# roysubhankar/dwt-domain-adaptation

Hardware: AMD Instinct MI355X
Metric: imgs_per_sec (higher is better)
Workload: dtype bf16; 1 GPU; model=resnet50-dwt-mec-3stream, global_batch=1536, seq_len=224, parallelism=dp1, per_domain_batch=512, group_size=4, whiten_mode=zca

## Files before the change

### dwt_amd/kernels/hip_ops.py

```python
from __future__ import annotations

import warnings
import torch

from . import dispatch

_GEN_G_MAX = 32
_warned = set()


def _whiten_layout(x, c, g):
    if x.dim() == 4 and x.is_contiguous(memory_format=torch.channels_last) \
            and not x.is_contiguous():
        if c % 64 == 0 and (c <= 256 or c % 256 == 0) and g in (2, 4):
            gw = min(c, 256) // g
            if gw > 0 and 256 % gw == 0:
                return "cl"
    return "nchw"


def _bn_cl_supported(c):
    if c % 4 != 0 or (c > 1024 and c % 1024 != 0):
        return False
    nch = min(c, 1024) // 4
    return 256 % nch == 0


def _bn_layout(x, c):
    if x.dim() == 2 and x.is_contiguous() and _bn_cl_supported(c):
        return "cl"
    if x.dim() == 4 and x.is_contiguous(memory_format=torch.channels_last) \
            and not x.is_contiguous() and _bn_cl_supported(c):
        return "cl"
    return "nchw"


def _warn_once(key, msg):
    if key not in _warned:
        _warned.add(key)
        warnings.warn(msg)


def _sync_world():
    import torch.distributed as dist
    if dist.is_available() and dist.is_initialized():
        return dist, dist.get_world_size()
    return None, 1


def _allreduce(t):
    import torch.distributed as dist
    dist.all_reduce(t)
    return t


def _ext():
    return dispatch.ext()


def _f32c(t):
    return t.detach().to(torch.float32).contiguous()


class _HipWhitenMulti(torch.autograd.Function):

    @staticmethod
    def forward(ctx, x, gamma, beta, running_means, running_vars, cfg,
                res=None):
        ext = _ext()
        parts = cfg["parts"]
        g = x.shape[1] // cfg["num_groups"]
        eps, momentum = cfg["eps"], cfg["momentum"]
        training, mode, relu = cfg["training"], cfg["mode"], cfg["relu"]
        track = cfg.get("track_running_stats", True)
        ns_iters = cfg.get("ns_iters", 7)
        use_batch = training or not track

        c = x.shape[1]
        layout = _whiten_layout(x, c, g)
        if layout == "nchw":
            x = x.contiguous()
        n, c, h, w = x.shape
        assert n % parts == 0,             f"batch {n} not divisible by {parts} domain branches"
        b = n // parts
        n_groups = c // g
        ng_all = parts * n_groups
        dev = x.device
        m_count = b * h * w

        has_affine = gamma is not None
        gflat = gamma.detach().reshape(c).contiguous() if has_affine else torch.empty(0, device=dev, dtype=x.dtype)
        bflat = beta.detach().reshape(c).contiguous() if has_affine else torch.empty(0, device=dev, dtype=x.dtype)

        stats_sync = cfg.get("stats_sync", False) and use_batch
        world = 1
        if stats_sync:
            _, world = _sync_world()
        ctx_count = m_count * world

        out = torch.empty_like(x)
        if use_batch:
            acc = torch.zeros(ng_all * (g + g * g), device=dev, dtype=torch.float32)
            mean = torch.empty(parts * c, device=dev, dtype=torch.float32)
            cov = torch.empty(ng_all, g, g, device=dev, dtype=torch.float32)
            if stats_sync:
                if layout == "cl":
                    ext.whiten_stats_partial_cl(x, acc, g, c, m_count, parts)
                else:
                    for p in range(parts):
                        ext.whiten_stats_partial(
                            x[p * b:(p + 1) * b],
                            acc[p * n_groups * (g + g * g):(p + 1) * n_groups * (g + g * g)], g)
                if world > 1:
                    _allreduce(acc)
                ext.whiten_stats_final(acc, mean, cov, g, ng_all, ctx_count)
            elif layout == "cl":
                ext.whiten_stats_cl(x, acc, mean, cov, g, c, m_count, parts)
            else:
                for p in range(parts):
                    ext.whiten_stats(x[p * b:(p + 1) * b],
                                     acc[p * n_groups * (g + g * g):(p + 1) * n_groups * (g + g * g)],
                                     mean[p * c:(p + 1) * c],
                                     cov[p * n_groups:(p + 1) * n_groups], g)
        else:
            mean = torch.stack([_f32c(running_means[p]).reshape(c)
                                for p in range(parts)]).reshape(-1).contiguous()
            cov = torch.stack([_f32c(running_vars[p]).reshape(n_groups, g, g)
                               for p in range(parts)]).reshape(ng_all, g, g).contiguous()
# ... 188 lines not shown
    c = x.shape[1]
    if kind == "whiten":
        return _whiten_layout(x, c, c // cfg["num_groups"]) == "cl"
    return _bn_layout(x, c) == "cl"


def whiten_join(x, identity, gamma, beta, running_means, running_vars, cfg):
    return _HipWhitenJoin.apply(x, identity, gamma, beta, running_means,
                                running_vars, cfg)


def batch_norm_join(x, identity, gamma, beta, running_means, running_vars, cfg):
    return _HipBatchNormJoin.apply(x, identity, gamma, beta, running_means,
                                   running_vars, cfg)


def whiten_multi(x, gamma, beta, running_means, running_vars, cfg):
    g = x.shape[1] // cfg["num_groups"]
    if g > _GEN_G_MAX or x.dtype not in (torch.float32, torch.bfloat16):
        _warn_once(("wh", g, x.dtype),
                   f"dwt_amd: whiten_multi g={g} dtype={x.dtype} uses the "
                   "torch path (HIP kernels cover g <= 32, fp32/bf16)")
        from ..ops.functional import WhitenMulti
        return WhitenMulti.apply(x, gamma, beta, running_means, running_vars, cfg)
    return _HipWhitenMulti.apply(x, gamma, beta, running_means, running_vars, cfg)


class _HipBatchNormMulti(torch.autograd.Function):
    @staticmethod
    def forward(ctx, x, gamma, beta, running_means, running_vars, cfg,
                res=None):
        ext = _ext()
        parts = cfg["parts"]
        eps, momentum = cfg["eps"], cfg["momentum"]
        training, relu = cfg["training"], cfg["relu"]
        track = cfg.get("track_running_stats", True)
        use_batch = training or not track

        spatial = x.dim() == 4
        c = x.shape[1]
        layout = _bn_layout(x, c)
        if layout == "nchw" or x.dim() == 2:
            x = x.contiguous()
        n = x.shape[0]
        assert n % parts == 0,             f"batch {n} not divisible by {parts} domain branches"
        b = n // parts
        dev = x.device
        cnt = (x.numel() // parts) // c

        has_affine = gamma is not None
        gflat = gamma.detach().reshape(c).contiguous() if has_affine else torch.empty(0, device=dev, dtype=x.dtype)
        bflat = beta.detach().reshape(c).contiguous() if has_affine else torch.empty(0, device=dev, dtype=x.dtype)

        stats_sync = cfg.get("stats_sync", False) and use_batch
        world = 1
        if stats_sync:
            _, world = _sync_world()
        cnt_total = cnt * world

        out = torch.empty_like(x)
        if use_batch:
            acc = torch.zeros(parts * 2 * c, device=dev, dtype=torch.float32)
            mean = torch.empty(parts * c, device=dev, dtype=torch.float32)
            istd = torch.empty(parts * c, device=dev, dtype=torch.float32)
            var_unb = torch.empty(parts * c, device=dev, dtype=torch.float32)
            if stats_sync:
                if layout == "cl":
                    ext.bn_stats_partial_cl(x, acc, c, cnt, parts)
                else:
                    for p in range(parts):
                        ext.bn_stats_partial(x[p * b:(p + 1) * b],
                                             acc[p * 2 * c:(p + 1) * 2 * c])
                if world > 1:
                    _allreduce(acc)
                ext.bn_stats_final(acc, mean, istd, var_unb, c, parts,
                                   cnt_total, eps)
            elif layout == "cl":
                ext.bn_stats_cl(x, acc, mean, istd, var_unb, c, cnt, eps, parts)
            else:
                for p in range(parts):
                    ext.bn_stats(x[p * b:(p + 1) * b],
                                 acc[p * 2 * c:(p + 1) * 2 * c],
                                 mean[p * c:(p + 1) * c],
                                 istd[p * c:(p + 1) * c],
                                 var_unb[p * c:(p + 1) * c], eps)
            if training and track and running_means is not None:
                with torch.no_grad():
                    for p in range(parts):
                        rm, rv = running_means[p], running_vars[p]
# ... 116 lines not shown
    @staticmethod
    def forward(ctx, x, identity, gamma, beta, running_means, running_vars,
                cfg):
        ctx.set_materialize_grads(False)
        res = identity.detach()
        y = _HipBatchNormMulti.forward(ctx, x, gamma, beta, running_means,
                                       running_vars, cfg, res=res)
        return y, y.view_as(y)

    @staticmethod
    def backward(ctx, ga, gb):
        if ga is None and gb is None:
            return (None,) * 7
        if ga is None:
            ga, gb = gb, None
        dx, gid, dgamma, dbeta = _HipBatchNormMulti.run_backward(
            ctx, ga, gb, join=True)
        return dx, gid, dgamma, dbeta, None, None, None


def batch_norm_multi(x, gamma, beta, running_means, running_vars, cfg):
    if x.dtype not in (torch.float32, torch.bfloat16):
        from ..ops.functional import BatchNormMulti
        return BatchNormMulti.apply(x, gamma, beta, running_means, running_vars, cfg)
    return _HipBatchNormMulti.apply(x, gamma, beta, running_means, running_vars, cfg)


class _HipMecLoss(torch.autograd.Function):
    @staticmethod
    def forward(ctx, x, y):
        ext = _ext()
        x32 = x.detach().to(torch.float32).contiguous()
        y32 = y.detach().to(torch.float32).contiguous()
        n, k = x32.shape
        lx = torch.empty_like(x32)
        ly = torch.empty_like(y32)
        amin = torch.empty(n, device=x.device, dtype=torch.int32)
        loss = torch.zeros(1, device=x.device, dtype=torch.float32)
        ext.mec_fwd(x32, y32, lx, ly, amin, loss)
        ctx.save_for_backward(lx, ly, amin)
        ctx.dtypes = (x.dtype, y.dtype)
        return loss[0]

    @staticmethod
    def backward(ctx, dloss):
        ext = _ext()
# ... 66 lines not shown
```

### dwt_amd/kernels/src/dwt_kernels.hip

```cpp

#include <torch/extension.h>
#include <ATen/cuda/CUDAContext.h>
#include <hip/hip_runtime.h>

#include <cstdint>

#define DEV_INLINE __device__ __forceinline__

namespace dwt {


DEV_INLINE float ldf(const float* p) { return *p; }
DEV_INLINE float ldf(const c10::BFloat16* p) {
  unsigned short u = *reinterpret_cast<const unsigned short*>(p);
  union { unsigned int i; float f; } v;
  v.i = static_cast<unsigned int>(u) << 16;
  return v.f;
}
DEV_INLINE void stf(float* p, float v) { *p = v; }
DEV_INLINE void stf(c10::BFloat16* p, float v) {
  union { unsigned int i; float f; } u;
  u.f = v;
  unsigned int lsb = (u.i >> 16) & 1u;
  unsigned int rounded = u.i + 0x7fffu + lsb;
// ... 3104 lines not shown
                     0, cur_stream(), q.data_ptr<float>(),
                     target.data_ptr<int64_t>(), gscale.data_ptr<float>(),
                     dx.data_ptr<float>(), N, K);
}

void entropy_bwd(Tensor q, Tensor hper, Tensor gscale, Tensor dx) {
  const int N = q.size(0), K = q.size(1);
  const int64_t total = (int64_t)N * K;
  hipLaunchKernelGGL(dwt::entropy_bwd_kernel,
                     dim3(elementwise_blocks(total, 256)), dim3(256), 0,
                     cur_stream(), q.data_ptr<float>(), hper.data_ptr<float>(),
                     gscale.data_ptr<float>(), dx.data_ptr<float>(), N, K);
}

}

void mfma_gemm(torch::Tensor a, torch::Tensor bt, torch::Tensor bias,
               torch::Tensor out, bool relu, bool has_bias);
void mfma_conv2d_fwd(torch::Tensor x, torch::Tensor wgt, torch::Tensor bias,
                     torch::Tensor out, int64_t N, int64_t H, int64_t W,
                     int64_t Cin, int64_t P, int64_t Q, int64_t Cout,
                     int64_t KH, int64_t KW, int64_t stride, int64_t pad,
                     bool relu, bool has_bias);
void mfma_conv2d_dgrad(torch::Tensor dy, torch::Tensor wd, torch::Tensor dx,
                       int64_t N, int64_t H, int64_t W, int64_t Cin,
                       int64_t P, int64_t Q, int64_t Cdy, int64_t KH,
                       int64_t KW, int64_t stride, int64_t pad);
void mfma_conv2d_wgrad(torch::Tensor dy, torch::Tensor x, torch::Tensor dw,
                       torch::Tensor ws, int64_t N, int64_t H, int64_t W,
                       int64_t Cin, int64_t P, int64_t Q, int64_t Cout,
                       int64_t KH, int64_t KW, int64_t stride, int64_t pad);

PYBIND11_MODULE(TORCH_EXTENSION_NAME, m) {
  m.def("mfma_gemm", &mfma_gemm);
  m.def("mfma_conv2d_fwd", &mfma_conv2d_fwd);
  m.def("mfma_conv2d_dgrad", &mfma_conv2d_dgrad);
  m.def("mfma_conv2d_wgrad", &mfma_conv2d_wgrad);
  m.def("whiten_stats", &whiten_stats);
  m.def("whiten_stats_partial", &whiten_stats_partial);
  m.def("whiten_stats_partial_cl", &whiten_stats_partial_cl);
  m.def("whiten_stats_final", &whiten_stats_final);
  m.def("bn_stats_partial", &bn_stats_partial);
  m.def("bn_stats_partial_cl", &bn_stats_partial_cl);
  m.def("bn_stats_final", &bn_stats_final);
  m.def("whiten_stats_cl", &whiten_stats_cl);
  m.def("whiten_apply_cl", &whiten_apply_cl);
  m.def("whiten_bwd_reduce_cl", &whiten_bwd_reduce_cl);
  m.def("whiten_bwd_apply_cl", &whiten_bwd_apply_cl);
  m.def("bn_stats_cl", &bn_stats_cl);
  m.def("bn_apply_cl", &bn_apply_cl);
  m.def("bn_bwd_reduce_cl", &bn_bwd_reduce_cl);
  m.def("bn_bwd_apply_cl", &bn_bwd_apply_cl);
  m.def("whiten_apply_res_cl", &whiten_apply_res_cl);
  m.def("bn_apply_res_cl", &bn_apply_res_cl);
  m.def("whiten_join_bwd_reduce_cl", &whiten_join_bwd_reduce_cl);
  m.def("bn_join_bwd_reduce_cl", &bn_join_bwd_reduce_cl);
  m.def("matfn_chol_fwd", &matfn_chol_fwd);
  m.def("matfn_chol_bwd", &matfn_chol_bwd);
// ... 26 lines not shown
```

### dwt_amd/kernels/src/mfma_conv.hip

```cpp

#include <torch/extension.h>
#include <ATen/cuda/CUDAContext.h>
#include <hip/hip_runtime.h>

#include <cstdint>

namespace dwtmm {

using bf16 = c10::BFloat16;
typedef __attribute__((ext_vector_type(8))) short short8;
typedef __attribute__((ext_vector_type(4))) float floatx4;

#define DEV_INLINE __device__ __forceinline__

constexpr int BM = 128, BN = 128, BK = 64;
constexpr int THREADS = 256;
constexpr int PAD_HALFS = 8;
constexpr int LDS_PITCH = BK + PAD_HALFS;

struct ConvParams {
  int N, H, W, Cin;
  int P, Q, Cout;
  int KH, KW, stride, pad;
  int64_t M;
// ... 300 lines not shown
        __syncthreads();
      }
    } else {
      __syncthreads();
    }
  }

  const int erow = (lane / 16) * 4;
  const int ecol = lane % 16;
#pragma unroll
  for (int i = 0; i < 4; ++i) {
#pragma unroll
    for (int r = 0; r < 4; ++r) {
      const int64_t m = m0 + wm + i * 16 + erow + r;
      if (m >= cp.M) continue;
#pragma unroll
      for (int j = 0; j < 4; ++j) {
        const int n = n0 + wn + j * 16 + ecol;
        if (n >= cp.Cout) continue;
        float v = acc[i][j][r];
        if (HAS_BIAS) v += bias[n];
        if (RELU) v = fmaxf(v, 0.f);
        *reinterpret_cast<unsigned short*>(out + m * cp.Cout + n) = f_to_bf16(v);
      }
    }
  }
}




constexpr int WBK = 64;
constexpr int WPITCH = WBK;

DEV_INLINE int wswz(int row) { return ((row >> 3) ^ row) & 7; }

template <bool ALIGNED_B, int WT>
__global__ __launch_bounds__(256, WT == 64 ? 4 : 3) void wgrad_splitk_kernel(
    const bf16* __restrict__ dy, const bf16* __restrict__ x,
    float* __restrict__ ws, ConvParams cp, int mtiles, int ntiles,
    int splitk, int64_t klen) {
  constexpr int NP = WT / 64;
  constexpr int NF = WT / 32;
  __shared__ unsigned short lds_a[WT * WPITCH];
  __shared__ unsigned short lds_b[WT * WPITCH];

// ... 361 lines not shown
                                                                   : dwtmm::A_CONV,
                                            decltype(reluc)::value,
                                            decltype(biasc)::value,
                                            decltype(pipec)::value,
                                            decltype(swzc)::value>),
          dim3(mtiles * ntiles), dim3(dwtmm::THREADS), 0, dwtmm_stream(),
          (const c10::BFloat16*)x.data_ptr(), (const c10::BFloat16*)wgt.data_ptr(),
          has_bias ? bias.data_ptr<float>() : nullptr,
          (c10::BFloat16*)out.data_ptr(), cp, mtiles, ntiles);
    };
    if (pipe) { if (swz) launch(std::true_type{}, std::true_type{});
                else launch(std::true_type{}, std::false_type{}); }
    else { if (swz) launch(std::false_type{}, std::true_type{});
           else launch(std::false_type{}, std::false_type{}); }
  };
  auto pick_rb = [&](auto fastc) {
    if (relu) { if (has_bias) run(fastc, std::true_type{}, std::true_type{});
                else run(fastc, std::true_type{}, std::false_type{}); }
    else { if (has_bias) run(fastc, std::false_type{}, std::true_type{});
           else run(fastc, std::false_type{}, std::false_type{}); }
  };
  if (gemm_fast) pick_rb(std::true_type{});
  else pick_rb(std::false_type{});
}


void mfma_conv2d_dgrad(Tensor dy, Tensor wd, Tensor dx, int64_t N, int64_t H,
                       int64_t W, int64_t Cin, int64_t P, int64_t Q,
                       int64_t Cdy, int64_t KH, int64_t KW, int64_t stride,
                       int64_t pad) {
  dwtmm::ConvParams cp{};
  cp.N = N; cp.H = H; cp.W = W; cp.Cin = Cin;
  cp.P = P; cp.Q = Q; cp.Cout = Cin;
  cp.KH = KH; cp.KW = KW; cp.stride = stride; cp.pad = pad;
  cp.Cdy = Cdy;
  cp.M = N * H * W;
  cp.K = KH * KW * Cdy;
  cp.cShift = log2_if_pow2(Cdy);
  const int mtiles = (cp.M + dwtmm::BM - 1) / dwtmm::BM;
  const int ntiles = (Cin + dwtmm::BN - 1) / dwtmm::BN;
  const bool gemm_fast = (KH == 1 && KW == 1 && stride == 1 && pad == 0 &&
                          Cdy % 8 == 0);
  const bool pipe = gemm_fast && cp.K >= 4 * dwtmm::BK;
  const bool swz = gemm_fast && ntiles >= 8 && mtiles * ntiles >= 16;
  auto launch = [&](auto modec, auto pipec, auto swzc) {
    hipLaunchKernelGGL(
// ... 93 lines not shown
```

### dwt_amd/models/resnet_dwt.py

```python
from __future__ import annotations

from typing import Dict, Optional

import torch
import torch.nn as nn

from ..ops.batch_norm import DomainBatchNorm2d
from ..ops.whitening import WhiteningScaleShift
from ..ops.pooling import MaxPool2dDWT, global_avg_pool
from .sites import norm_site


def _conv_cls():
    import os
    if os.environ.get("DWT_AMD_CONV") == "hip":
        from ..ops.mfma import MFMAConv2d
        return MFMAConv2d
    return nn.Conv2d


def conv3x3(cin, cout, stride=1):
    return _conv_cls()(cin, cout, kernel_size=3, stride=stride, padding=1, bias=False)


def conv1x1(cin, cout, stride=1):
    return _conv_cls()(cin, cout, kernel_size=1, stride=stride, bias=False)


def _get(bn_dict: Optional[Dict], key: str):
    if bn_dict is None:
        return None
    return bn_dict.get(key)


def _make_wh_branches(planes, group_size, bn_dict, prefix, mode):
    branches = []
    for _ in range(3):
        rm = _get(bn_dict, f"{prefix}.wh.running_mean")
        rv = _get(bn_dict, f"{prefix}.wh.running_variance")
        branches.append(WhiteningScaleShift(
            planes, group_size,
            running_mean=rm.clone() if rm is not None else None,
            running_variance=rv.clone() if rv is not None else None,
            affine=False, mode=mode))
    g = _get(bn_dict, f"{prefix}.gamma")
    b = _get(bn_dict, f"{prefix}.beta")
    gamma = nn.Parameter(g.clone() if g is not None else torch.ones(planes, 1, 1))
    beta = nn.Parameter(b.clone() if b is not None else torch.zeros(planes, 1, 1))
    return branches, gamma, beta
# ... 39 lines not shown
            site(planes * self.expansion, "bn3")

        self.downsample = downsample
        self.stride = stride
        if downsample is not None:
            dpre = f"layer{layer}.0.downsample_bn"
            if use_wh:
                (self.downsample_bns, self.downsample_bnt, self.downsample_bnt_aug), \
                    self.downsample_gamma, self.downsample_beta = _make_wh_branches(
                        planes * self.expansion, group_size, bn_dict, dpre, whiten_mode)
            else:
                (self.downsample_bns, self.downsample_bnt, self.downsample_bnt_aug), \
                    self.downsample_gamma, self.downsample_beta = _make_bn_branches(
                        planes * self.expansion, bn_dict, dpre)

    def forward(self, x):
        return self.forward_pair(x, x)[0]

    def forward_pair(self, x_main, x_id):
        tr = self.training
        x = x_main
        identity = x_id

        out = self.conv1(x)
        out = norm_site(out, [self.bns1, self.bnt1, self.bnt1_aug],
                        self.gamma1, self.beta1, training=tr, relu=True)
        out = self.conv2(out)
        out = norm_site(out, [self.bns2, self.bnt2, self.bnt2_aug],
                        self.gamma2, self.beta2, training=tr, relu=True)
        out = self.conv3(out)

        if self.downsample is not None:
            identity = self.downsample(x)
            identity = norm_site(
                identity,
                [self.downsample_bns, self.downsample_bnt, self.downsample_bnt_aug],
                self.downsample_gamma, self.downsample_beta, training=tr, relu=False)

        return norm_site(out, [self.bns3, self.bnt3, self.bnt3_aug],
                         self.gamma3, self.beta3, training=tr, relu=True,
                         residual=identity)


class _Stage(nn.Sequential):

    def forward(self, x):
        a = b = x
        for block in self:
            a, b = block.forward_pair(a, b)
        return a


class ResNetDWT(nn.Module):
    def __init__(self, block, layers, bn_dict=None, num_classes=65,
                 group_size=4, whiten_mode="chol"):
        super().__init__()
        self.inplanes = 64
        self.whiten_mode = whiten_mode

        self.conv1 = _conv_cls()(3, 64, kernel_size=7, stride=2, padding=3, bias=False)
        (self.bns1, self.bnt1, self.bnt1_aug), self.gamma1, self.beta1 = \
            _make_wh_branches(64, group_size, bn_dict, "bn1", whiten_mode)
        self.maxpool = MaxPool2dDWT(kernel_size=3, stride=2, padding=1)
        self.layer1 = self._make_layer(block, 64, layers[0], bn_dict, layer=1,
# ... 57 lines not shown
```

### dwt_amd/models/sites.py

```python
from __future__ import annotations

from typing import Optional, Sequence

import torch
import torch.nn as nn

from ..ops import functional as Fdwt
from ..ops.whitening import WhiteningScaleShift, WTransform2d
from ..ops.batch_norm import _DomainBatchNorm


def _wh_of(mod: nn.Module) -> WTransform2d:
    return mod.wh if isinstance(mod, WhiteningScaleShift) else mod


def norm_site(
    x: torch.Tensor,
    branches: Sequence[nn.Module],
    gamma: Optional[torch.Tensor],
    beta: Optional[torch.Tensor],
    training: bool,
    relu: bool,
    eval_branch: int = 1,
    residual: Optional[torch.Tensor] = None,
):
    if residual is not None:
        assert relu, "a residual join applies its ReLU after the add"
    first = branches[0]
    if training:
        use = list(branches)
        parts = len(use)
    else:
        use = [branches[min(eval_branch, len(branches) - 1)]]
        parts = 1

    if isinstance(first, (WhiteningScaleShift, WTransform2d)):
        whs = [_wh_of(b) for b in use]
        w0 = whs[0]
        kw = dict(parts=parts, num_groups=w0.num_groups, eps=w0.eps,
                  momentum=w0.momentum, training=training, mode=w0.mode,
                  track_running_stats=w0.track_running_stats)
        rms = [w.running_mean for w in whs]
        rvs = [w.running_variance for w in whs]
        if residual is not None:
            return Fdwt.norm_join("whiten", x, residual, gamma, beta, rms, rvs,
                                  **kw)
        return Fdwt.whiten_multi(x, gamma, beta, rms, rvs, relu=relu, **kw)

    if isinstance(first, (_DomainBatchNorm, nn.modules.batchnorm._BatchNorm)):
        momentum = first.momentum if first.momentum is not None else 0.0
        if training and first.track_running_stats:
            for b in use:
                if b.num_batches_tracked is not None:
                    b.num_batches_tracked += 1
            if first.momentum is None:
                momentum = 1.0 / first.num_batches_tracked.item()
        spatial = x.dim() == 4
        gshape = (-1, 1, 1) if spatial else (1, -1)
        gamma = gamma.reshape(gshape) if gamma is not None else None
        beta = beta.reshape(gshape) if beta is not None else None
        rms = [b.running_mean for b in use] if first.track_running_stats else None
        rvs = [b.running_var for b in use] if first.track_running_stats else None
        kw = dict(parts=parts, eps=first.eps, momentum=momentum,
                  training=training,
                  track_running_stats=first.track_running_stats)
        if residual is not None:
            return Fdwt.norm_join("bn", x, residual, gamma, beta, rms, rvs, **kw)
        return Fdwt.batch_norm_multi(x, gamma, beta, rms, rvs, relu=relu, **kw)

    raise TypeError(f"unsupported norm branch type {type(first)}")
```

### dwt_amd/ops/functional.py

```python
from __future__ import annotations

import os
from typing import List, Optional, Sequence

import torch
import torch.nn.functional as F

from . import oracle




def matfn_chol_forward(cov_s: torch.Tensor):
    ell = torch.linalg.cholesky(cov_s)
    eye = torch.eye(ell.shape[-1], dtype=ell.dtype, device=ell.device).expand_as(ell)
    w = torch.linalg.solve_triangular(ell, eye, upper=False)
    return w, ell


def matfn_chol_backward(w: torch.Tensor, ell: torch.Tensor, w_bar: torch.Tensor):
    l_bar = torch.tril(-w.transpose(-1, -2) @ w_bar @ w.transpose(-1, -2))
    s = ell.transpose(-1, -2) @ l_bar
    phi = torch.tril(s)
    phi = phi - 0.5 * torch.diag_embed(phi.diagonal(dim1=-2, dim2=-1))
# ... 231 lines not shown
               training=training, mode=mode, relu=relu, ns_iters=ns_iters,
               track_running_stats=track_running_stats)
    if os.environ.get("DWT_AMD_STATS_SYNC") == "1":
        cfg["stats_sync"] = True
    return cfg


def whiten_multi(
    x: torch.Tensor,
    gamma: Optional[torch.Tensor],
    beta: Optional[torch.Tensor],
    running_means: Optional[Sequence[torch.Tensor]],
    running_vars: Optional[Sequence[torch.Tensor]],
    *,
    parts: int,
    num_groups: int,
    eps: float = 1e-3,
    momentum: float = 0.1,
    training: bool = True,
    mode: str = "chol",
    relu: bool = False,
    ns_iters: int = 7,
    track_running_stats: bool = True,
) -> torch.Tensor:
    cfg = _whiten_cfg(parts=parts, num_groups=num_groups, eps=eps,
                      momentum=momentum, training=training, mode=mode,
                      relu=relu, ns_iters=ns_iters,
                      track_running_stats=track_running_stats)
    if x.is_cuda:
        from ..kernels import dispatch
        if dispatch.available():
            return dispatch.whiten_multi(x, gamma, beta, running_means, running_vars, cfg)
        dispatch.require_or_warn("whiten_multi")
    return WhitenMulti.apply(x, gamma, beta, running_means, running_vars, cfg)




class BatchNormMulti(torch.autograd.Function):

    @staticmethod
    def forward(ctx, x, gamma, beta, running_means, running_vars, cfg):
        parts = cfg["parts"]
        eps = cfg["eps"]
        momentum = cfg["momentum"]
        training = cfg["training"]
        relu = cfg["relu"]
        track = cfg.get("track_running_stats", True)
        use_batch = training or not track

        spatial = x.dim() == 4
        n = x.shape[0]
        c = x.shape[1]
        b = n // parts
# ... 105 lines not shown
    relu: bool = False,
    track_running_stats: bool = True,
) -> dict:
    cfg = dict(parts=parts, eps=eps, momentum=momentum, training=training,
               relu=relu, track_running_stats=track_running_stats)
    if os.environ.get("DWT_AMD_STATS_SYNC") == "1":
        cfg["stats_sync"] = True
    return cfg


def batch_norm_multi(
    x: torch.Tensor,
    gamma: Optional[torch.Tensor],
    beta: Optional[torch.Tensor],
    running_means: Optional[Sequence[torch.Tensor]],
    running_vars: Optional[Sequence[torch.Tensor]],
    *,
    parts: int,
    eps: float = 1e-5,
    momentum: float = 0.1,
    training: bool = True,
    relu: bool = False,
    track_running_stats: bool = True,
) -> torch.Tensor:
    cfg = _bn_cfg(parts=parts, eps=eps, momentum=momentum, training=training,
                  relu=relu, track_running_stats=track_running_stats)
    if x.is_cuda:
        from ..kernels import dispatch
        if dispatch.available():
            return dispatch.batch_norm_multi(x, gamma, beta, running_means, running_vars, cfg)
        dispatch.require_or_warn("batch_norm_multi")
    return BatchNormMulti.apply(x, gamma, beta, running_means, running_vars, cfg)




class MecLossFn(torch.autograd.Function):

    @staticmethod
    def forward(ctx, x, y):
        ct = torch.float64 if x.dtype == torch.float64 else torch.float32
        lx = F.log_softmax(x.to(ct), dim=1)
        ly = F.log_softmax(y.to(ct), dim=1)
        per = -0.5 * (lx + ly)
        vals, idx = per.min(dim=1)
        ctx.save_for_backward(lx, ly, idx)
        ctx.dtypes = (x.dtype, y.dtype)
        return vals.mean()

    @staticmethod
    def backward(ctx, dloss):
        lx, ly, idx = ctx.saved_tensors
# ... 89 lines not shown
        return d, d


def add_relu(a: torch.Tensor, b: torch.Tensor) -> torch.Tensor:
    return AddReluFn.apply(a, b)


def fused_join_enabled() -> bool:
    return os.environ.get("DWT_AMD_FUSED_JOIN", "1") != "0"


def norm_join(
    kind: str,
    x: torch.Tensor,
    identity: torch.Tensor,
    gamma: Optional[torch.Tensor],
    beta: Optional[torch.Tensor],
    running_means: Optional[Sequence[torch.Tensor]],
    running_vars: Optional[Sequence[torch.Tensor]],
    **kw,
):
    assert kind in ("whiten", "bn"), kind
    kw = dict(kw, relu=False)
    if x.is_cuda and fused_join_enabled():
        from ..kernels import dispatch
        if dispatch.available():
            from ..kernels import hip_ops
            cfg = _whiten_cfg(**kw) if kind == "whiten" else _bn_cfg(**kw)
            if hip_ops.join_supported(kind, x, identity, cfg):
                fn = hip_ops.whiten_join if kind == "whiten" \
                    else hip_ops.batch_norm_join
                return fn(x, identity, gamma, beta, running_means,
                          running_vars, cfg)
    multi = whiten_multi if kind == "whiten" else batch_norm_multi
    y = add_relu(multi(x, gamma, beta, running_means, running_vars, **kw),
                 identity)
    return y, y


def ce_loss(logits: torch.Tensor, target: torch.Tensor) -> torch.Tensor:
    if logits.is_cuda:
        from ..kernels import dispatch
        if dispatch.available():
            return dispatch.ce_loss(logits, target)
        dispatch.require_or_warn("ce_loss")
    return F.nll_loss(F.log_softmax(logits.float(), dim=1), target)
```

### dwt_amd/ops/mfma.py

```python
from __future__ import annotations

from typing import Optional

import torch
import torch.nn as nn
import torch.nn.functional as F


def _ext():
    from ..kernels import dispatch
    return dispatch.ext()


def _pad_k(t: torch.Tensor) -> torch.Tensor:
    k = t.shape[1]
    if k % 8 == 0:
        return t
    return F.pad(t, (0, 8 - k % 8))


def mfma_gemm(a: torch.Tensor, bt: torch.Tensor,
              bias: Optional[torch.Tensor] = None, relu: bool = False):
    assert a.dtype == torch.bfloat16 and bt.dtype == torch.bfloat16
    a = _pad_k(a.contiguous())
# ... 50 lines not shown
        x4[:, 3] = 0
        x4[:, :3] = x
        w4 = torch.empty(cout, 4, kh, kw, device=x.device, dtype=weight.dtype,
                         memory_format=torch.channels_last)
        w4[:, 3] = 0
        w4[:, :3] = weight.detach()
        x, weight, cin = x4, w4, 4
    p = (h + 2 * padding - kh) // stride + 1
    q = (w + 2 * padding - kw) // stride + 1
    out = torch.empty(n, cout, p, q, device=x.device, dtype=torch.bfloat16,
                      memory_format=torch.channels_last)
    wgt = weight
    if not wgt.is_contiguous(memory_format=torch.channels_last):
        wgt = wgt.contiguous(memory_format=torch.channels_last)
    has_bias = bias is not None
    b32 = bias.detach().float().contiguous() if has_bias else torch.empty(0, device=x.device)
    if (kh * kw * cin) % 8 != 0 and not (kh == 1 and kw == 1 and stride == 1 and padding == 0):
        pass
    _ext().mfma_conv2d_fwd(x, wgt, b32, out, n, h, w, cin, p, q, cout,
                           kh, kw, stride, padding, relu, has_bias)
    return out


def conv2d_dgrad(dy: torch.Tensor, weight: torch.Tensor, in_shape,
                 stride: int = 1, padding: int = 0) -> torch.Tensor:
    n, cin, h, w = in_shape
    cout, _, kh, kw = weight.shape
    p, q = dy.shape[2], dy.shape[3]
    dyc = dy.contiguous(memory_format=torch.channels_last)
    wv = weight.permute(0, 2, 3, 1)
    wd = wv.permute(3, 1, 2, 0).contiguous()
    dx = torch.empty(n, cin, h, w, device=dy.device, dtype=torch.bfloat16,
                     memory_format=torch.channels_last)
    _ext().mfma_conv2d_dgrad(dyc, wd, dx, n, h, w, cin, p, q, cout,
                             kh, kw, stride, padding)
    return dx


class _MFMAConv2dFn(torch.autograd.Function):

    @staticmethod
    def forward(ctx, x, weight, bias, stride, padding):
        out = conv2d_fwd(x, weight, bias=bias, stride=stride, padding=padding)
        ctx.save_for_backward(x, weight)
        ctx.meta = (stride, padding, bias is not None)
        return out
# ... 78 lines not shown
```

### dwt_amd/ops/oracle.py

```python
from __future__ import annotations

import torch
import torch.nn.functional as F



def channel_mean(x: torch.Tensor) -> torch.Tensor:
    return x.mean(dim=(0, 2, 3), keepdim=True)


def grouped_cov(xn: torch.Tensor, num_groups: int) -> torch.Tensor:
    n, c, h, w = xn.shape
    g = c // num_groups
    t = xn.permute(1, 0, 2, 3).reshape(num_groups, g, n * h * w)
    return torch.bmm(t, t.transpose(1, 2)) / t.shape[-1]


def shrink_cov(cov: torch.Tensor, eps: float) -> torch.Tensor:
    g = cov.shape[-1]
    eye = torch.eye(g, dtype=cov.dtype, device=cov.device)
    return (1.0 - eps) * cov + eps * eye




def whiten_matrix_chol(cov_shrunk: torch.Tensor) -> torch.Tensor:
    ell = torch.linalg.cholesky(cov_shrunk)
    return torch.linalg.solve_triangular(
        ell, torch.eye(ell.shape[-1], dtype=ell.dtype, device=ell.device).expand_as(ell),
        upper=False,
    )


def whiten_matrix_ns(cov_shrunk: torch.Tensor, iters: int = 7) -> torch.Tensor:
    g = cov_shrunk.shape[-1]
    eye = torch.eye(g, dtype=cov_shrunk.dtype, device=cov_shrunk.device).expand_as(cov_shrunk)
    s = cov_shrunk.diagonal(dim1=-2, dim2=-1).sum(-1).clamp_min(1e-30)
    s_ = s.view(-1, 1, 1)
# ... 71 lines not shown
```

Measured before the change: 8927 images/sec.

## Fuse BN/whitening statistics accumulation into 1x1 conv epilogue

Adds an MFMA 1x1 convolution kernel that accumulates per-branch BN sums or g=4 whitening sums and lower-triangular cross products in its epilogue. The normalization layers then only finalize from the precomputed accumulator instead of re-reading the conv output for a separate stats pass. This saves one full read of large activations per eligible 1x1 conv. In exchange, the GEMM is a custom kernel that may be slower than the existing conv path, and the epilogue adds LDS atomics and global atomics.

```diff
diff --git a/dwt_amd/kernels/hip_ops.py b/dwt_amd/kernels/hip_ops.py
--- a/dwt_amd/kernels/hip_ops.py
+++ b/dwt_amd/kernels/hip_ops.py
@@ -12,11 +12,16 @@
 def _whiten_layout(x, c, g):
     if x.dim() == 4 and x.is_contiguous(memory_format=torch.channels_last) \
             and not x.is_contiguous():
-        if c % 64 == 0 and (c <= 256 or c % 256 == 0) and g in (2, 4):
-            gw = min(c, 256) // g
-            if gw > 0 and 256 % gw == 0:
-                return "cl"
+        if whiten_cl_supported(c, g):
+            return "cl"
     return "nchw"
+
+
+def whiten_cl_supported(c, g):
+    if c % 64 == 0 and (c <= 256 or c % 256 == 0) and g in (2, 4):
+        gw = min(c, 256) // g
+        return gw > 0 and 256 % gw == 0
+    return False
 
 
 def _bn_cl_supported(c):
@@ -62,12 +67,22 @@
     return t.detach().to(torch.float32).contiguous()
 
 
+def _usable_stats_acc(acc, x, layout, training, numel):
+    if acc is None or not training or layout != "cl" or x.dim() != 4:
+        return None
+    if acc.dtype != torch.float32 or acc.device != x.device \
+            or acc.numel() != numel or not acc.is_contiguous():
+        return None
+    return acc.detach().reshape(-1)
+
+
 class _HipWhitenMulti(torch.autograd.Function):
 
     @staticmethod
     def forward(ctx, x, gamma, beta, running_means, running_vars, cfg,
                 res=None):
         ext = _ext()
+        stats_acc = cfg.pop("stats_acc", None)
         parts = cfg["parts"]
         g = x.shape[1] // cfg["num_groups"]
         eps, momentum = cfg["eps"], cfg["momentum"]
@@ -100,10 +115,18 @@
 
         out = torch.empty_like(x)
         if use_batch:
-            acc = torch.zeros(ng_all * (g + g * g), device=dev, dtype=torch.float32)
+            acc = _usable_stats_acc(stats_acc, x, layout, training,
+                                    ng_all * (g + g * g))
+            pre = acc is not None
+            if not pre:
+                acc = torch.zeros(ng_all * (g + g * g), device=dev, dtype=torch.float32)
             mean = torch.empty(parts * c, device=dev, dtype=torch.float32)
             cov = torch.empty(ng_all, g, g, device=dev, dtype=torch.float32)
-            if stats_sync:
+            if pre:
+                if stats_sync and world > 1:
+                    _allreduce(acc)
+                ext.whiten_stats_final(acc, mean, cov, g, ng_all, ctx_count)
+            elif stats_sync:
                 if layout == "cl":
                     ext.whiten_stats_partial_cl(x, acc, g, c, m_count, parts)
                 else:
@@ -338,6 +361,7 @@
                    f"dwt_amd: whiten_multi g={g} dtype={x.dtype} uses the "
                    "torch path (HIP kernels cover g <= 32, fp32/bf16)")
         from ..ops.functional import WhitenMulti
+        cfg.pop("stats_acc", None)
         return WhitenMulti.apply(x, gamma, beta, running_means, running_vars, cfg)
     return _HipWhitenMulti.apply(x, gamma, beta, running_means, running_vars, cfg)
 
@@ -347,6 +371,7 @@
     def forward(ctx, x, gamma, beta, running_means, running_vars, cfg,
                 res=None):
         ext = _ext()
+        stats_acc = cfg.pop("stats_acc", None)
         parts = cfg["parts"]
         eps, momentum = cfg["eps"], cfg["momentum"]
         training, relu = cfg["training"], cfg["relu"]
@@ -376,11 +401,20 @@
 
         out = torch.empty_like(x)
         if use_batch:
-            acc = torch.zeros(parts * 2 * c, device=dev, dtype=torch.float32)
+            acc = _usable_stats_acc(stats_acc, x, layout, training,
+                                    parts * 2 * c)
+            pre = acc is not None
+            if not pre:
+                acc = torch.zeros(parts * 2 * c, device=dev, dtype=torch.float32)
             mean = torch.empty(parts * c, device=dev, dtype=torch.float32)
             istd = torch.empty(parts * c, device=dev, dtype=torch.float32)
             var_unb = torch.empty(parts * c, device=dev, dtype=torch.float32)
-            if stats_sync:
+            if pre:
+                if stats_sync and world > 1:
+                    _allreduce(acc)
+                ext.bn_stats_final(acc, mean, istd, var_unb, c, parts,
+                                   cnt_total, eps)
+            elif stats_sync:
                 if layout == "cl":
                     ext.bn_stats_partial_cl(x, acc, c, cnt, parts)
                 else:
@@ -543,6 +577,7 @@
 def batch_norm_multi(x, gamma, beta, running_means, running_vars, cfg):
     if x.dtype not in (torch.float32, torch.bfloat16):
         from ..ops.functional import BatchNormMulti
+        cfg.pop("stats_acc", None)
         return BatchNormMulti.apply(x, gamma, beta, running_means, running_vars, cfg)
     return _HipBatchNormMulti.apply(x, gamma, beta, running_means, running_vars, cfg)
 
diff --git a/dwt_amd/kernels/src/dwt_kernels.hip b/dwt_amd/kernels/src/dwt_kernels.hip
--- a/dwt_amd/kernels/src/dwt_kernels.hip
+++ b/dwt_amd/kernels/src/dwt_kernels.hip
@@ -3150,6 +3150,9 @@
                      int64_t Cin, int64_t P, int64_t Q, int64_t Cout,
                      int64_t KH, int64_t KW, int64_t stride, int64_t pad,
                      bool relu, bool has_bias);
+void conv1x1_stats(torch::Tensor x, torch::Tensor wgt, torch::Tensor out,
+                   torch::Tensor acc, int64_t kind, int64_t g, int64_t parts,
+                   int64_t max_workgroups);
 void mfma_conv2d_dgrad(torch::Tensor dy, torch::Tensor wd, torch::Tensor dx,
                        int64_t N, int64_t H, int64_t W, int64_t Cin,
                        int64_t P, int64_t Q, int64_t Cdy, int64_t KH,
@@ -3162,6 +3165,7 @@
 PYBIND11_MODULE(TORCH_EXTENSION_NAME, m) {
   m.def("mfma_gemm", &mfma_gemm);
   m.def("mfma_conv2d_fwd", &mfma_conv2d_fwd);
+  m.def("conv1x1_stats", &conv1x1_stats);
   m.def("mfma_conv2d_dgrad", &mfma_conv2d_dgrad);
   m.def("mfma_conv2d_wgrad", &mfma_conv2d_wgrad);
   m.def("whiten_stats", &whiten_stats);
diff --git a/dwt_amd/kernels/src/mfma_conv.hip b/dwt_amd/kernels/src/mfma_conv.hip
--- a/dwt_amd/kernels/src/mfma_conv.hip
+++ b/dwt_amd/kernels/src/mfma_conv.hip
@@ -346,6 +346,224 @@
         if (HAS_BIAS) v += bias[n];
         if (RELU) v = fmaxf(v, 0.f);
         *reinterpret_cast<unsigned short*>(out + m * cp.Cout + n) = f_to_bf16(v);
+      }
+    }
+  }
+}
+
+
+enum StatsKind { STATS_BN = 0, STATS_WHITEN4 = 1 };
+
+constexpr int C_PITCH = BN + PAD_HALFS;
+
+template <int CTRL>
+DEV_INLINE float quad_bcast(float v) {
+  union { int i; float f; } a, b;
+  a.f = v;
+  b.i = __builtin_amdgcn_mov_dpp(a.i, CTRL, 0xf, 0xf, true);
+  return b.f;
+}
+
+DEV_INLINE void load_rows(const bf16* __restrict__ base, const int (&off)[4],
+                          int nrows, int K, int k0, StageRegs& rg) {
+  const int t = threadIdx.x;
+#pragma unroll
+  for (int c = 0; c < 4; ++c) {
+    const int idx = t + c * THREADS;
+    const int row = idx / (BK / 8);
+    const int kc = (idx % (BK / 8)) * 8;
+    if (row < nrows && k0 + kc < K)
+      rg.c[c] = *reinterpret_cast<const uint4*>(base + off[c] + k0);
+    else
+      rg.c[c] = make_uint4(0, 0, 0, 0);
+  }
+}
+
+template <bool PIPE, int KIND>
+__global__ __launch_bounds__(THREADS, PIPE ? 2 : 3) void conv1x1_stats_kernel(
+    const bf16* __restrict__ x, const bf16* __restrict__ wgt,
+    bf16* __restrict__ out, float* __restrict__ acc, ConvParams cp,
+    int mtiles, int ntiles, int tiles_per_part, int nlanes, int runs) {
+  constexpr int TILE = BM * LDS_PITCH;
+  constexpr int NBUF = PIPE ? 2 : 1;
+  constexpr int NV = KIND == STATS_BN ? 2 : 5;
+  __shared__ __attribute__((aligned(16))) unsigned short lds[NBUF * 2 * TILE];
+  __shared__ float sacc[BN * NV];
+  static_assert(BM * C_PITCH <= 2 * TILE, "C staging must fit the A/B storage");
+
+  int bid = blockIdx.x;
+  {
+    const int nwg = gridDim.x;
+    const int nx = 8;
+    const int qq = nwg / nx, rr = nwg % nx;
+    const int xcd = bid % nx, idx = bid / nx;
+    bid = (xcd < rr ? xcd * (qq + 1) : rr * (qq + 1) + (xcd - rr) * qq) + idx;
+  }
+  const int nlane = bid % nlanes;
+  const int run = bid / nlanes;
+  const int mt_begin = (int)((int64_t)run * mtiles / runs);
+  const int mt_end = (int)((int64_t)(run + 1) * mtiles / runs);
+
+  const int wave = threadIdx.x / 64;
+  const int lane = threadIdx.x % 64;
+  const int wm = (wave / 2) * 64;
+  const int wn = (wave % 2) * 64;
+  const int frag_row = lane % 16;
+  const int frag_koff = (lane / 16) * 8;
+  const int erow = (lane / 16) * 4;
+  const int ecol = lane % 16;
+  const int nk = (cp.K + BK - 1) / BK;
+
+  int off[4];
+#pragma unroll
+  for (int q = 0; q < 4; ++q) {
+    const int idx = threadIdx.x + q * THREADS;
+    off[q] = (idx / (BK / 8)) * cp.K + (idx % (BK / 8)) * 8;
+  }
+
+  for (int k = threadIdx.x; k < BN * NV; k += THREADS) sacc[k] = 0.f;
+  __syncthreads();
+
+  for (int nt = nlane; nt < ntiles; nt += nlanes) {
+    const int n0 = nt * BN;
+    const bf16* wb = wgt + (int64_t)n0 * cp.K;
+    const int brows = cp.Cout - n0 < BN ? cp.Cout - n0 : BN;
+    for (int mt = mt_begin; mt < mt_end; ++mt) {
+      const int64_t m0 = (int64_t)mt * BM;
+
+      floatx4 c[4][4];
+#pragma unroll
+      for (int i = 0; i < 4; ++i)
+#pragma unroll
+        for (int j = 0; j < 4; ++j) c[i][j] = (floatx4){0.f, 0.f, 0.f, 0.f};
+
+      StageRegs ra, rb;
+      const bf16* xa = x + m0 * cp.K;
+      const int arows = (int)(cp.M - m0 < BM ? cp.M - m0 : BM);
+      if (PIPE) {
+        load_rows(xa, off, arows, cp.K, 0, ra);
+        load_rows(wb, off, brows, cp.K, 0, rb);
+        write_tile(ra, lds);
+        write_tile(rb, lds + TILE);
+        __syncthreads();
+      }
+      for (int t = 0; t < nk; ++t) {
+        const int cur = PIPE ? (t & 1) : 0;
+        unsigned short* la = lds + (2 * cur) * TILE;
+        unsigned short* lb = la + TILE;
+        if (PIPE) {
+          if (t + 1 < nk) {
+            load_rows(xa, off, arows, cp.K, (t + 1) * BK, ra);
+            load_rows(wb, off, brows, cp.K, (t + 1) * BK, rb);
+          }
+        } else {
+          load_rows(xa, off, arows, cp.K, t * BK, ra);
+          load_rows(wb, off, brows, cp.K, t * BK, rb);
+          write_tile(ra, la);
+          write_tile(rb, lb);
+          __syncthreads();
+        }
+#pragma unroll
+        for (int ks = 0; ks < BK; ks += 32) {
+          short8 afrag[4], bfrag[4];
+#pragma unroll
+          for (int i = 0; i < 4; ++i) {
+            afrag[i] = *reinterpret_cast<const short8*>(
+                la + (wm + i * 16 + frag_row) * LDS_PITCH + ks + frag_koff);
+            bfrag[i] = *reinterpret_cast<const short8*>(
+                lb + (wn + i * 16 + frag_row) * LDS_PITCH + ks + frag_koff);
+          }
+#pragma unroll
+          for (int i = 0; i < 4; ++i)
+#pragma unroll
+            for (int j = 0; j < 4; ++j)
+              c[i][j] = __builtin_amdgcn_mfma_f32_16x16x32_bf16(
+                  afrag[i], bfrag[j], c[i][j], 0, 0, 0);
+        }
+        if (PIPE) {
+          __syncthreads();
+          if (t + 1 < nk) {
+            const int nxt = cur ^ 1;
+            write_tile(ra, lds + (2 * nxt) * TILE);
+            write_tile(rb, lds + (2 * nxt + 1) * TILE);
+            __syncthreads();
+          }
+        } else {
+          __syncthreads();
+        }
+      }
+
+#pragma unroll
+      for (int j = 0; j < 4; ++j) {
+        const int col = wn + j * 16 + ecol;
+        float s = 0.f, p0 = 0.f, p1 = 0.f, p2 = 0.f, p3 = 0.f;
+#pragma unroll
+        for (int i = 0; i < 4; ++i) {
+#pragma unroll
+          for (int r = 0; r < 4; ++r) {
+            const unsigned short u = f_to_bf16(c[i][j][r]);
+            const float v = bf16_to_f(u);
+            lds[(wm + i * 16 + erow + r) * C_PITCH + col] = u;
+            s += v;
+            if (KIND == STATS_BN) {
+              p0 += v * v;
+            } else {
+              p0 += v * quad_bcast<0x00>(v);
+              p1 += v * quad_bcast<0x55>(v);
+              p2 += v * quad_bcast<0xAA>(v);
+              p3 += v * quad_bcast<0xFF>(v);
+            }
+          }
+        }
+        if (KIND == STATS_BN) {
+          atomicAdd(&sacc[col], s);
+          atomicAdd(&sacc[BN + col], p0);
+        } else {
+          float* mine = sacc + col * NV;
+          atomicAdd(&mine[0], s);
+          atomicAdd(&mine[1], p0);
+          atomicAdd(&mine[2], p1);
+          atomicAdd(&mine[3], p2);
+          atomicAdd(&mine[4], p3);
+        }
+      }
+      __syncthreads();
+
+#pragma unroll
+      for (int q = 0; q < (BM * BN / 8) / THREADS; ++q) {
+        const int idx = threadIdx.x + q * THREADS;
+        const int row = idx / (BN / 8);
+        const int cc = (idx % (BN / 8)) * 8;
+        const int64_t m = m0 + row;
+        const int n = n0 + cc;
+        if (m < cp.M && n < cp.Cout)
+          *reinterpret_cast<uint4*>(out + m * cp.Cout + n) =
+              *reinterpret_cast<const uint4*>(lds + row * C_PITCH + cc);
+      }
+      __syncthreads();
+
+      const int part = mt / tiles_per_part;
+      if (mt + 1 == mt_end || (mt + 1) / tiles_per_part != part) {
+        for (int k = threadIdx.x; k < BN * NV; k += THREADS) {
+          const float v = sacc[k];
+          sacc[k] = 0.f;
+          if (KIND == STATS_BN) {
+            const int which = k / BN;
+            const int n = n0 + k % BN;
+            if (n < cp.Cout)
+              atomicAdd(acc + ((int64_t)part * 2 + which) * cp.Cout + n, v);
+          } else {
+            const int n = n0 + k / NV;
+            const int e = k % NV;
+            const int i = n & 3;
+            if (n < cp.Cout && e <= i + 1) {
+              const int64_t grp = (int64_t)part * (cp.Cout / 4) + n / 4;
+              const int slot = e == 0 ? i : 4 + i * 4 + (e - 1);
+              atomicAdd(acc + grp * 20 + slot, v);
+            }
+          }
+        }
+        __syncthreads();
       }
     }
   }
@@ -753,6 +971,65 @@
   };
   if (gemm_fast) pick_rb(std::true_type{});
   else pick_rb(std::false_type{});
+}
+
+
+void conv1x1_stats(Tensor x, Tensor wgt, Tensor out, Tensor acc, int64_t kind,
+                   int64_t g, int64_t parts, int64_t max_workgroups) {
+  TORCH_CHECK(x.scalar_type() == at::kBFloat16 &&
+              wgt.scalar_type() == at::kBFloat16 &&
+              out.scalar_type() == at::kBFloat16 &&
+              acc.scalar_type() == at::kFloat, "conv1x1_stats: dtypes");
+  TORCH_CHECK(x.is_cuda() && wgt.is_cuda() && out.is_cuda() && acc.is_cuda());
+  TORCH_CHECK(wgt.dim() >= 2 && acc.is_contiguous());
+  const int64_t Cout = wgt.size(0);
+  const int64_t Cin = wgt.numel() / Cout;
+  TORCH_CHECK(Cin % 8 == 0 && Cout % 8 == 0, "conv1x1_stats: C % 8");
+  TORCH_CHECK(x.numel() % Cin == 0);
+  const int64_t M = x.numel() / Cin;
+  TORCH_CHECK(out.numel() == M * Cout);
+  TORCH_CHECK(parts >= 1 && M % parts == 0 && (M / parts) % dwtmm::BM == 0,
+              "conv1x1_stats: rows per branch must be a multiple of ",
+              dwtmm::BM);
+  TORCH_CHECK(kind == dwtmm::STATS_BN || (kind == dwtmm::STATS_WHITEN4 && g == 4),
+              "conv1x1_stats: BN or whitening with g = 4 only");
+  const int64_t acc_n = kind == dwtmm::STATS_BN ? parts * 2 * Cout
+                                                : parts * (Cout / 4) * 20;
+  TORCH_CHECK(acc.numel() == acc_n, "conv1x1_stats: acc size");
+  TORCH_CHECK(M / dwtmm::BM < (int64_t)1 << 31);
+
+  dwtmm::ConvParams cp{};
+  cp.M = M; cp.K = (int)Cin; cp.Cout = (int)Cout;
+  const int mtiles = (int)(M / dwtmm::BM);
+  const int ntiles = (int)((Cout + dwtmm::BN - 1) / dwtmm::BN);
+  const bool pipe = cp.K >= 4 * dwtmm::BK;
+  int64_t maxwg = max_workgroups;
+  if (maxwg <= 0) {
+    static const int cus =
+        at::cuda::getCurrentDeviceProperties()->multiProcessorCount;
+    maxwg = (int64_t)cus * (pipe ? 2 : 3);
+  }
+  const int nlanes = (int)std::min<int64_t>(maxwg, ntiles);
+  const int runs = (int)std::max<int64_t>(
+      1, std::min<int64_t>(maxwg / nlanes, mtiles));
+  auto launch = [&](auto pipec, auto kindc) {
+    hipLaunchKernelGGL(
+        (dwtmm::conv1x1_stats_kernel<decltype(pipec)::value,
+                                     decltype(kindc)::value>),
+        dim3(nlanes * runs), dim3(dwtmm::THREADS), 0, dwtmm_stream(),
+        (const c10::BFloat16*)x.data_ptr(), (const c10::BFloat16*)wgt.data_ptr(),
+        (c10::BFloat16*)out.data_ptr(), acc.data_ptr<float>(), cp, mtiles,
+        ntiles, (int)(M / parts / dwtmm::BM), nlanes, runs);
+  };
+  using KBN = std::integral_constant<int, dwtmm::STATS_BN>;
+  using KWH = std::integral_constant<int, dwtmm::STATS_WHITEN4>;
+  if (kind == dwtmm::STATS_BN) {
+    if (pipe) launch(std::true_type{}, KBN{});
+    else launch(std::false_type{}, KBN{});
+  } else {
+    if (pipe) launch(std::true_type{}, KWH{});
+    else launch(std::false_type{}, KWH{});
+  }
 }
 
 
diff --git a/dwt_amd/models/resnet_dwt.py b/dwt_amd/models/resnet_dwt.py
--- a/dwt_amd/models/resnet_dwt.py
+++ b/dwt_amd/models/resnet_dwt.py
@@ -25,6 +25,15 @@
 
 def conv1x1(cin, cout, stride=1):
     return _conv_cls()(cin, cout, kernel_size=1, stride=stride, bias=False)
+
+
+def _conv_with_stats(conv, x, branches, training):
+    from ..ops import mfma
+    route = mfma.conv_stats_route(conv, x, branches, training)
+    if route is None:
+        return conv(x), None
+    kind, g, parts = route
+    return mfma.conv1x1_stats(x, conv.weight, kind, g, parts)
 
 
 def _get(bn_dict: Optional[Dict], key: str):
@@ -110,24 +119,30 @@
         x = x_main
         identity = x_id
 
-        out = self.conv1(x)
-        out = norm_site(out, [self.bns1, self.bnt1, self.bnt1_aug],
-                        self.gamma1, self.beta1, training=tr, relu=True)
+        site1 = [self.bns1, self.bnt1, self.bnt1_aug]
+        out, acc = _conv_with_stats(self.conv1, x, site1, tr)
+        out = norm_site(out, site1, self.gamma1, self.beta1, training=tr,
+                        relu=True, stats_acc=acc)
         out = self.conv2(out)
         out = norm_site(out, [self.bns2, self.bnt2, self.bnt2_aug],
                         self.gamma2, self.beta2, training=tr, relu=True)
-        out = self.conv3(out)
+        site3 = [self.bns3, self.bnt3, self.bnt3_aug]
+        out, acc = _conv_with_stats(self.conv3, out, site3, tr)
 
         if self.downsample is not None:
-            identity = self.downsample(x)
+            dsite = [self.downsample_bns, self.downsample_bnt,
+                     self.downsample_bnt_aug]
+            if len(self.downsample) == 1:
+                identity, dacc = _conv_with_stats(self.downsample[0], x,
+                                                  dsite, tr)
+            else:
+                identity, dacc = self.downsample(x), None
             identity = norm_site(
-                identity,
-                [self.downsample_bns, self.downsample_bnt, self.downsample_bnt_aug],
-                self.downsample_gamma, self.downsample_beta, training=tr, relu=False)
-
-        return norm_site(out, [self.bns3, self.bnt3, self.bnt3_aug],
-                         self.gamma3, self.beta3, training=tr, relu=True,
-                         residual=identity)
+                identity, dsite, self.downsample_gamma, self.downsample_beta,
+                training=tr, relu=False, stats_acc=dacc)
+
+        return norm_site(out, site3, self.gamma3, self.beta3, training=tr,
+                         relu=True, residual=identity, stats_acc=acc)
 
 
 class _Stage(nn.Sequential):
diff --git a/dwt_amd/models/sites.py b/dwt_amd/models/sites.py
--- a/dwt_amd/models/sites.py
+++ b/dwt_amd/models/sites.py
@@ -23,9 +23,12 @@
     relu: bool,
     eval_branch: int = 1,
     residual: Optional[torch.Tensor] = None,
+    stats_acc: Optional[torch.Tensor] = None,
 ):
     if residual is not None:
         assert relu, "a residual join applies its ReLU after the add"
+    if not training:
+        stats_acc = None
     first = branches[0]
     if training:
         use = list(branches)
@@ -39,7 +42,8 @@
         w0 = whs[0]
         kw = dict(parts=parts, num_groups=w0.num_groups, eps=w0.eps,
                   momentum=w0.momentum, training=training, mode=w0.mode,
-                  track_running_stats=w0.track_running_stats)
+                  track_running_stats=w0.track_running_stats,
+                  stats_acc=stats_acc)
         rms = [w.running_mean for w in whs]
         rvs = [w.running_variance for w in whs]
         if residual is not None:
@@ -63,7 +67,8 @@
         rvs = [b.running_var for b in use] if first.track_running_stats else None
         kw = dict(parts=parts, eps=first.eps, momentum=momentum,
                   training=training,
-                  track_running_stats=first.track_running_stats)
+                  track_running_stats=first.track_running_stats,
+                  stats_acc=stats_acc)
         if residual is not None:
             return Fdwt.norm_join("bn", x, residual, gamma, beta, rms, rvs, **kw)
         return Fdwt.batch_norm_multi(x, gamma, beta, rms, rvs, relu=relu, **kw)
diff --git a/dwt_amd/ops/functional.py b/dwt_amd/ops/functional.py
--- a/dwt_amd/ops/functional.py
+++ b/dwt_amd/ops/functional.py
@@ -277,6 +277,7 @@
     relu: bool = False,
     ns_iters: int = 7,
     track_running_stats: bool = True,
+    stats_acc: Optional[torch.Tensor] = None,
 ) -> torch.Tensor:
     cfg = _whiten_cfg(parts=parts, num_groups=num_groups, eps=eps,
                       momentum=momentum, training=training, mode=mode,
@@ -285,6 +286,8 @@
     if x.is_cuda:
         from ..kernels import dispatch
         if dispatch.available():
+            if stats_acc is not None:
+                cfg["stats_acc"] = stats_acc
             return dispatch.whiten_multi(x, gamma, beta, running_means, running_vars, cfg)
         dispatch.require_or_warn("whiten_multi")
     return WhitenMulti.apply(x, gamma, beta, running_means, running_vars, cfg)
@@ -436,12 +439,15 @@
     training: bool = True,
     relu: bool = False,
     track_running_stats: bool = True,
+    stats_acc: Optional[torch.Tensor] = None,
 ) -> torch.Tensor:
     cfg = _bn_cfg(parts=parts, eps=eps, momentum=momentum, training=training,
                   relu=relu, track_running_stats=track_running_stats)
     if x.is_cuda:
         from ..kernels import dispatch
         if dispatch.available():
+            if stats_acc is not None:
+                cfg["stats_acc"] = stats_acc
             return dispatch.batch_norm_multi(x, gamma, beta, running_means, running_vars, cfg)
         dispatch.require_or_warn("batch_norm_multi")
     return BatchNormMulti.apply(x, gamma, beta, running_means, running_vars, cfg)
@@ -577,18 +583,22 @@
 ):
     assert kind in ("whiten", "bn"), kind
     kw = dict(kw, relu=False)
+    stats_acc = kw.pop("stats_acc", None)
     if x.is_cuda and fused_join_enabled():
         from ..kernels import dispatch
         if dispatch.available():
             from ..kernels import hip_ops
             cfg = _whiten_cfg(**kw) if kind == "whiten" else _bn_cfg(**kw)
             if hip_ops.join_supported(kind, x, identity, cfg):
+                if stats_acc is not None:
+                    cfg["stats_acc"] = stats_acc
                 fn = hip_ops.whiten_join if kind == "whiten" \
                     else hip_ops.batch_norm_join
                 return fn(x, identity, gamma, beta, running_means,
                           running_vars, cfg)
     multi = whiten_multi if kind == "whiten" else batch_norm_multi
-    y = add_relu(multi(x, gamma, beta, running_means, running_vars, **kw),
+    y = add_relu(multi(x, gamma, beta, running_means, running_vars,
+                       stats_acc=stats_acc, **kw),
                  identity)
     return y, y
 
diff --git a/dwt_amd/ops/mfma.py b/dwt_amd/ops/mfma.py
--- a/dwt_amd/ops/mfma.py
+++ b/dwt_amd/ops/mfma.py
@@ -96,6 +96,129 @@
     return out
 
 
+
+STATS_TILE_M = 128
+_STATS_KINDS = {"bn": 0, "whiten": 1}
+
+
+def fused_conv_stats_enabled() -> bool:
+    import os
+    return os.environ.get("DWT_AMD_FUSED_CONV_STATS", "1") != "0"
+
+
+def stats_acc_numel(kind: str, c: int, parts: int, g: int = 4) -> int:
+    if kind == "bn":
+        return parts * 2 * c
+    return parts * (c // g) * (g + g * g)
+
+
+def conv_stats_shape_ok(m: int, cin: int, cout: int) -> bool:
+    del m
+    return cin >= _ROUTE_MIN_C and cout >= _ROUTE_MIN_C
+
+
+_ROUTE_MIN_C = 128
+
+
+def conv_stats_route(conv, x: torch.Tensor, branches, training: bool):
+    if not training or not fused_conv_stats_enabled():
+        return None
+    if not (x.is_cuda and x.dtype == torch.bfloat16 and x.dim() == 4
+            and x.is_contiguous(memory_format=torch.channels_last)):
+        return None
+    if type(conv) is not nn.Conv2d or conv.bias is not None \
+            or conv.kernel_size != (1, 1) or conv.stride != (1, 1) \
+            or conv.padding != (0, 0) or conv.dilation != (1, 1) \
+            or conv.groups != 1 or conv.weight.dtype != torch.bfloat16:
+        return None
+    from ..kernels import dispatch
+    if not dispatch.available():
+        return None
+    from ..kernels import hip_ops
+    from .whitening import WhiteningScaleShift, WTransform2d
+    from .batch_norm import _DomainBatchNorm
+    n, cin, h, w = x.shape
+    cout = conv.out_channels
+    parts = len(branches)
+    first = branches[0]
+    if isinstance(first, (WhiteningScaleShift, WTransform2d)):
+        wh = first.wh if isinstance(first, WhiteningScaleShift) else first
+        g = cout // wh.num_groups
+        if g != 4 or not hip_ops.whiten_cl_supported(cout, g):
+            return None
+        kind = "whiten"
+    elif isinstance(first, _DomainBatchNorm):
+        if not hip_ops._bn_cl_supported(cout):
+            return None
+        kind, g = "bn", 0
+    else:
+        return None
+    if h * w == 1 or cout == 1:
+        return None
+    if cin % 8 or cout % 8 or n % parts \
+            or (n // parts * h * w) % STATS_TILE_M:
+        return None
+    if not conv_stats_shape_ok(n * h * w, cin, cout):
+        return None
+    return kind, g, parts
+
+
+class _Conv1x1StatsFn(torch.autograd.Function):
+
+    calls = 0
+
+    @staticmethod
+    def forward(ctx, x, weight, kind, g, parts, max_workgroups):
+        n, cin, h, w = x.shape
+        cout = weight.shape[0]
+        out = torch.empty(n, cout, h, w, device=x.device, dtype=torch.bfloat16,
+                          memory_format=torch.channels_last)
+        acc = torch.zeros(stats_acc_numel(kind, cout, parts), device=x.device,
+                          dtype=torch.float32)
+        wgt = weight.detach().reshape(cout, cin).contiguous()
+        _ext().conv1x1_stats(x, wgt, out, acc, _STATS_KINDS[kind], g, parts,
+                             max_workgroups)
+        _Conv1x1StatsFn.calls += 1
+        ctx.save_for_backward(x, weight)
+        ctx.mark_non_differentiable(acc)
+        return out, acc
+
+    @staticmethod
+    def backward(ctx, dout, _dacc):
+        x, weight = ctx.saved_tensors
+        dx, dw, _ = torch.ops.aten.convolution_backward(
+            dout, x, weight, None, [1, 1], [0, 0], [1, 1], False, [0, 0], 1,
+            [ctx.needs_input_grad[0], True, False])
+        return dx, dw, None, None, None, None
+
+
+def conv1x1_stats(x: torch.Tensor, weight: torch.Tensor, kind: str,
+                  g: int = 4, parts: int = 3, max_workgroups: int = 0):
+    assert kind in _STATS_KINDS, kind
+    if not _conv1x1_stats_applies(x, weight, kind, g, parts):
+        return F.conv2d(x, weight), None
+    return _Conv1x1StatsFn.apply(x, weight, kind, g, parts, max_workgroups)
+
+
+def _conv1x1_stats_applies(x, weight, kind, g, parts) -> bool:
+    if not (x.is_cuda and x.dim() == 4 and x.dtype == torch.bfloat16
+            and weight.dtype == torch.bfloat16
+            and x.is_contiguous(memory_format=torch.channels_last)):
+        return False
+    if weight.dim() != 4 or weight.shape[2:] != (1, 1) \
+            or weight.shape[1] != x.shape[1]:
+        return False
+    n, cin, h, w = x.shape
+    cout = weight.shape[0]
+    if kind == "whiten" and g != 4:
+        return False
+    if cin % 8 or cout % 8 or parts < 1 or n % parts \
+            or (n // parts * h * w) % STATS_TILE_M:
+        return False
+    from ..kernels import dispatch
+    return dispatch.available()
+
+
 def conv2d_dgrad(dy: torch.Tensor, weight: torch.Tensor, in_shape,
                  stride: int = 1, padding: int = 0) -> torch.Tensor:
     n, cin, h, w = in_shape
diff --git a/dwt_amd/ops/oracle.py b/dwt_amd/ops/oracle.py
--- a/dwt_amd/ops/oracle.py
+++ b/dwt_amd/ops/oracle.py
@@ -14,6 +14,18 @@
     g = c // num_groups
     t = xn.permute(1, 0, 2, 3).reshape(num_groups, g, n * h * w)
     return torch.bmm(t, t.transpose(1, 2)) / t.shape[-1]
+
+
+def stats_acc_reference(out: torch.Tensor, kind: str, parts: int, g: int = 4,
+                        dtype=torch.float64) -> torch.Tensor:
+    c = out.shape[1]
+    v = out.detach().to(dtype).permute(0, 2, 3, 1).reshape(parts, -1, c)
+    if kind == "bn":
+        return torch.stack([v.sum(1), (v * v).sum(1)], dim=1).reshape(-1)
+    t = v.reshape(parts, v.shape[1], c // g, g)
+    sums = t.sum(1)
+    pm = torch.tril(torch.einsum("pmgi,pmgj->pgij", t, t))
+    return torch.cat([sums, pm.reshape(parts, c // g, g * g)], dim=2).reshape(-1)
 
 
 def shrink_cov(cov: torch.Tensor, eps: float) -> torch.Tensor:
```

New measurement: 9134 images/sec (median of 6 runs). +2.3%, better.
